# BatsResearch/menghini-neurips23-code

Measured on AMD Instinct MI355X. Metric: images/sec CLIP ViT-B/16 encode+prompt-step, higher is better.
Workload: dtype f16

## Files before the change

### menghini-neurips23-code_amd/csrc/attention_split.hip

```cpp
#include <math.h>

#include "common.h"

__device__ __forceinline__ int vt_index_fwd_s(int key, int d) { return vt_index(key, ((d >> 2) & 3) * 16 + (d >> 4) * 4 + (d & 3)); }

__device__ __forceinline__ void split8(const f32x4 a, const f32x4 b, half8& hi, half8& lo) {
    half4 h0, l0, h1, l1;
    split_f16x4(a, h0, l0);
    split_f16x4(b, h1, l1);
    hi = (half8){h0[0], h0[1], h0[2], h0[3], h1[0], h1[1], h1[2], h1[3]};
    lo = (half8){l0[0], l0[1], l0[2], l0[3], l1[0], l1[1], l1[2], l1[3]};
}

template <int KVC, bool CAUSAL, int NW>
__global__ __launch_bounds__(NW * 64) void attn_fwd_split_kernel(const float* __restrict__ qkv, half_t* __restrict__ out, int S, int H) {
    constexpr int SP = KVC * 32;
    constexpr float LOG2E = 1.4426950408889634f;
    constexpr float INV = 1.0f / (float)GRIP_SPLIT_LO_SCALE;
    extern __shared__ __attribute__((aligned(16))) char smem[];
    half_t* Kh = (half_t*)smem;
    half_t* Kl = Kh + SP * 64;
    half_t* Vh = Kl + SP * 64;
    half_t* Vl = Vh + SP * 64;

    const int tid = threadIdx.x, lane = tid & 63, wave = tid >> 6;
    const int D = H * 64;
    const int b = blockIdx.x / H, h = blockIdx.x - b * H;
    const size_t ld = (size_t)3 * D;
    const float* base = qkv + (size_t)b * S * ld + h * 64;
    const int li = lane & 15, lg = lane >> 4;
    const int n_qt = (S + 15) >> 4;

    for (int idx = tid; idx < SP * 8; idx += NW * 64) {
        const int row = idx >> 3, chunk = idx & 7;
        f32x4 a = {0.f, 0.f, 0.f, 0.f}, c = {0.f, 0.f, 0.f, 0.f};
        if (row < S) {
            const f32x4* p = (const f32x4*)(base + (size_t)row * ld + D + chunk * 8);
            a = p[0];
            c = p[1];
        }
        half8 hi, lo;
        split8(a, c, hi, lo);
        const int o = row * 64 + ((chunk ^ (row & 7)) * 8);
        *(half8*)(Kh + o) = hi;
        *(half8*)(Kl + o) = lo;
    }
    for (int idx = tid; idx < ((SP / 2 + 31) / 32) * 256; idx += NW * 64) {
        const int lane_rp = idx & 31, chunk = ((idx >> 5) & 1) + 2 * ((idx >> 6) & 3), rblk = idx >> 8;
        const int r0 = 2 * (rblk * 32 + lane_rp);
        if (r0 >= SP) continue;
        f32x4 z = {0.f, 0.f, 0.f, 0.f};
        f32x4 a0 = z, a1 = z, b0 = z, b1 = z;
        if (r0 < S) { const f32x4* p = (const f32x4*)(base + (size_t)r0 * ld + 2 * D + chunk * 8); a0 = p[0]; a1 = p[1]; }
        if (r0 + 1 < S) { const f32x4* p = (const f32x4*)(base + (size_t)(r0 + 1) * ld + 2 * D + chunk * 8); b0 = p[0]; b1 = p[1]; }
        half8 h0, l0, h1, l1;
        split8(a0, a1, h0, l0);
        split8(b0, b1, h1, l1);
#pragma unroll
        for (int j = 0; j < 8; ++j) {
            const int o = vt_index_fwd_s(r0, chunk * 8 + j);
            *(half2v*)(Vh + o) = (half2v){h0[j], h1[j]};
            *(half2v*)(Vl + o) = (half2v){l0[j], l1[j]};
        }
    }
    __syncthreads();

    for (int qt = wave; qt < n_qt; qt += NW) {
        asm volatile("" ::: "memory");
        const int qrow = qt * 16 + li;
        const int qr = qrow < S ? qrow : S - 1;
        half8 qh[2], ql[2];
#pragma unroll
        for (int kk = 0; kk < 2; ++kk) {
            const f32x4* p = (const f32x4*)(base + (size_t)qr * ld + (kk * 4 + lg) * 8);
            split8(p[0] * 0.125f, p[1] * 0.125f, qh[kk], ql[kk]);
        }
        f32x4 sc[2 * KVC];
        float m = -INFINITY;
#pragma unroll
        for (int t = 0; t < 2 * KVC; ++t) {
            f32x4 acc = {0.f, 0.f, 0.f, 0.f}, cor = {0.f, 0.f, 0.f, 0.f};
#pragma unroll
            for (int kk = 0; kk < 2; ++kk) {
                const int o = (t * 16 + li) * 64 + (((kk * 4 + lg) ^ (lane & 7)) * 8);
                const half8 kh = *(const half8*)(Kh + o), kl = *(const half8*)(Kl + o);
                acc = __builtin_amdgcn_mfma_f32_16x16x32_f16(kh, qh[kk], acc, 0, 0, 0);
                cor = __builtin_amdgcn_mfma_f32_16x16x32_f16(kl, qh[kk], cor, 0, 0, 0);
                cor = __builtin_amdgcn_mfma_f32_16x16x32_f16(kh, ql[kk], cor, 0, 0, 0);
            }
            acc += cor * INV;
            if (CAUSAL || t >= 2 * (KVC - 1)) {
#pragma unroll
                for (int r = 0; r < 4; ++r) {
                    const int kv = t * 16 + lg * 4 + r;
                    if (kv >= S || (CAUSAL && kv > qrow)) acc[r] = -INFINITY;
                }
            }
            m = fmaxf(fmaxf(fmaxf(m, acc[0]), fmaxf(acc[1], acc[2])), acc[3]);
            sc[t] = acc;
        }
        m = fmaxf(m, __shfl_xor(m, 16));
        m = fmaxf(m, __shfl_xor(m, 32));
        const float m2 = m * LOG2E;
#pragma unroll
        for (int t = 0; t < 2 * KVC; ++t)
#pragma unroll
            for (int r = 0; r < 4; ++r) sc[t][r] = __builtin_amdgcn_exp2f(__builtin_fmaf(sc[t][r], LOG2E, -m2));

        const half8 ones = {1, 1, 1, 1, 1, 1, 1, 1};
        f32x4 sum_h = {0.f, 0.f, 0.f, 0.f}, sum_l = {0.f, 0.f, 0.f, 0.f};
        f32x4 o[4], oc[4];
#pragma unroll
        for (int nf = 0; nf < 4; ++nf) { o[nf] = (f32x4){0.f, 0.f, 0.f, 0.f}; oc[nf] = (f32x4){0.f, 0.f, 0.f, 0.f}; }
#pragma unroll
        for (int c = 0; c < KVC; ++c) {
            half8 ph, pl;
            split8(sc[2 * c], sc[2 * c + 1], ph, pl);
#pragma unroll
            for (int nf = 0; nf < 4; ++nf) {
                const int vo = (c * 4 + nf) * 512 + (lg * 16 + (li ^ lg)) * 8;
                const half8 vh = *(const half8*)(Vh + vo), vl = *(const half8*)(Vl + vo);
                o[nf] = __builtin_amdgcn_mfma_f32_16x16x32_f16(vh, ph, o[nf], 0, 0, 0);
                oc[nf] = __builtin_amdgcn_mfma_f32_16x16x32_f16(vl, ph, oc[nf], 0, 0, 0);
                oc[nf] = __builtin_amdgcn_mfma_f32_16x16x32_f16(vh, pl, oc[nf], 0, 0, 0);
            }
            sum_h = __builtin_amdgcn_mfma_f32_16x16x32_f16(ones, ph, sum_h, 0, 0, 0);
            sum_l = __builtin_amdgcn_mfma_f32_16x16x32_f16(ones, pl, sum_l, 0, 0, 0);
        }
        if (qrow < S) {
            const float inv = 1.0f / (sum_h[0] + sum_l[0] * INV);
            half_t* orow = out + (size_t)((size_t)b * S + qrow) * 2 * D;
            const int col = h * 64 + lg * 16;
            half_t* op = orow + (col >> 5) * 64 + (col & 31);
            half8 hi0, lo0, hi1, lo1;
            split8((o[0] + oc[0] * INV) * inv, (o[1] + oc[1] * INV) * inv, hi0, lo0);
            split8((o[2] + oc[2] * INV) * inv, (o[3] + oc[3] * INV) * inv, hi1, lo1);
            *(half8*)op = hi0;
            *(half8*)(op + 8) = hi1;
            *(half8*)(op + 32) = lo0;
            *(half8*)(op + 40) = lo1;
        }
    }
}

bool attention_split_supported(int S) { return S >= 1 && S <= 320; }

int launch_attention_fwd_split(const float* qkv, void* out, int B, int S, int H, int causal, hipStream_t s) {
    GRIP_REQUIRE(attention_split_supported(S) && B >= 1 && H >= 1, "attention_split: bad shape B=%d S=%d H=%d (S <= 320)", B, S, H);
    const int kvc = (S + 31) / 32;
    const size_t lds = (size_t)4 * kvc * 32 * 64 * sizeof(half_t);
#define GRIP_ATT_CASE(K)                                                                                                                     \
    case K: {                                                                                                                                \
        static bool configured = false;                                                                                                      \
        if (!configured) {                                                                                                                   \
            GRIP_CHECK_HIP(hipFuncSetAttribute((const void*)attn_fwd_split_kernel<K, false, (K >= 4 ? 8 : 4)>, hipFuncAttributeMaxDynamicSharedMemorySize, (int)lds)); \
            GRIP_CHECK_HIP(hipFuncSetAttribute((const void*)attn_fwd_split_kernel<K, true, (K >= 4 ? 8 : 4)>, hipFuncAttributeMaxDynamicSharedMemorySize, (int)lds));  \
            configured = true;                                                                                                               \
        }                                                                                                                                    \
        if (causal) hipLaunchKernelGGL((attn_fwd_split_kernel<K, true, (K >= 4 ? 8 : 4)>), dim3(B * H), dim3((K >= 4 ? 8 : 4) * 64), lds, s, qkv, (half_t*)out, S, H); \
        else hipLaunchKernelGGL((attn_fwd_split_kernel<K, false, (K >= 4 ? 8 : 4)>), dim3(B * H), dim3((K >= 4 ? 8 : 4) * 64), lds, s, qkv, (half_t*)out, S, H);       \
    } break;
    switch (kvc) {
        GRIP_ATT_CASE(1) GRIP_ATT_CASE(2) GRIP_ATT_CASE(3) GRIP_ATT_CASE(4) GRIP_ATT_CASE(5)
        GRIP_ATT_CASE(6) GRIP_ATT_CASE(7) GRIP_ATT_CASE(8) GRIP_ATT_CASE(9) GRIP_ATT_CASE(10)
        default: GRIP_REQUIRE(false, "attention_split: S = %d out of range", S);
    }
#undef GRIP_ATT_CASE
    GRIP_CHECK_HIP(hipGetLastError());
    return GRIP_OK;
}
```

### menghini-neurips23-code_amd/csrc/common.h

```cpp
#pragma once
#include <hip/hip_runtime.h>
#include <stdint.h>
#include <stdio.h>
#include <string.h>

#include "host_common.h"
#include "gemm_plan.h"

typedef _Float16 half_t;
typedef half_t half8 __attribute__((ext_vector_type(8)));
typedef half_t half4 __attribute__((ext_vector_type(4)));
typedef half_t half2v __attribute__((ext_vector_type(2)));
typedef float f32x4 __attribute__((ext_vector_type(4)));

typedef half_t resid_t;

#define AS1 __attribute__((address_space(1)))
#define AS3 __attribute__((address_space(3)))

#define GRIP_CHECK_HIP(expr)                                                                   \
    do {                                                                                       \
        hipError_t _e = (expr);                                                                \
        if (_e != hipSuccess) {                                                                \
            grip_set_error("%s:%d %s -> %s", __FILE__, __LINE__, #expr, hipGetErrorString(_e)); \
// ... 11 lines not shown
    return (((c * 4 + (d >> 4)) * 64 + lg * 16 + ((d & 15) ^ lg)) * 8) + e;
}

#define LN_EPS 1e-5f
#define MAX_NV 8

__device__ __forceinline__ float wave_sum(float v) {
#define GRIP_DPP_ADD(ctrl) v += __builtin_bit_cast(float, __builtin_amdgcn_update_dpp(0, __builtin_bit_cast(int, v), ctrl, 0xF, 0xF, true))
    GRIP_DPP_ADD(0xB1);
    GRIP_DPP_ADD(0x4E);
    GRIP_DPP_ADD(0x141);
    GRIP_DPP_ADD(0x140);
#undef GRIP_DPP_ADD
    const int b = __builtin_bit_cast(int, v);
    const float r0 = __builtin_bit_cast(float, __builtin_amdgcn_readlane(b, 0)), r1 = __builtin_bit_cast(float, __builtin_amdgcn_readlane(b, 16));
    const float r2 = __builtin_bit_cast(float, __builtin_amdgcn_readlane(b, 32)), r3 = __builtin_bit_cast(float, __builtin_amdgcn_readlane(b, 48));
    return (r0 + r1) + (r2 + r3);
}
__device__ __forceinline__ float row16_sum(float v) {
#define GRIP_DPP_ADD(ctrl) v += __builtin_bit_cast(float, __builtin_amdgcn_update_dpp(0, __builtin_bit_cast(int, v), ctrl, 0xF, 0xF, true))
    GRIP_DPP_ADD(0xB1);
    GRIP_DPP_ADD(0x4E);
    GRIP_DPP_ADD(0x141);
    GRIP_DPP_ADD(0x140);
#undef GRIP_DPP_ADD
    return v;
}

__device__ __forceinline__ f32x4 load4(const float* p, int i) { return ((const f32x4*)p)[i]; }
__device__ __forceinline__ f32x4 load4(const half_t* p, int i) {
    const half4 h = ((const half4*)p)[i];
    return (f32x4){(float)h[0], (float)h[1], (float)h[2], (float)h[3]};
}
__device__ __forceinline__ void store4(float* p, int i, f32x4 v) { ((f32x4*)p)[i] = v; }
__device__ __forceinline__ void store4(half_t* p, int i, f32x4 v) { ((half4*)p)[i] = (half4){(half_t)v[0], (half_t)v[1], (half_t)v[2], (half_t)v[3]}; }
#ifndef GRIP_SPLIT_LO_SCALE
#define GRIP_SPLIT_LO_SCALE 1
#endif
#define SP1_W_SCALE 256.0f
__device__ __forceinline__ float quick_gelu_exact_s(float x) { return x * __builtin_amdgcn_rcpf(1.0f + __builtin_amdgcn_exp2f(-1.702f * 1.4426950408889634f * x)); }
struct SplitRow { half_t* p; };
__device__ __forceinline__ void split_f16x4(f32x4 v, half4& hi, half4& lo) {
#pragma unroll
    for (int e = 0; e < 4; ++e) {
        float x = v[e];
        asm volatile("" : "+v"(x));
        const half_t h = (half_t)x;
        hi[e] = h;
        lo[e] = (half_t)((x - (float)h) * (float)GRIP_SPLIT_LO_SCALE);
    }
}
__device__ __forceinline__ void store4(SplitRow r, int i, f32x4 v) {
    half4 hi, lo;
    split_f16x4(v, hi, lo);
    half_t* o = r.p + (i >> 3) * 64 + (i & 7) * 4;
    *(half4*)o = hi;
    *(half4*)(o + 32) = lo;
}

template <int NV>
__device__ __forceinline__ void ln_normalize(f32x4 (&v)[NV], int lane, int d4, int d, float& mean, float& rstd) {
#pragma clang fp contract(off)
    float s = 0.f;
#pragma unroll
    for (int i = 0; i < NV; ++i)
        if (lane + 64 * i < d4) s += v[i][0] + v[i][1] + v[i][2] + v[i][3];
    mean = wave_sum(s) / (float)d;
    float q = 0.f;
#pragma unroll
    for (int i = 0; i < NV; ++i)
        if (lane + 64 * i < d4) {
            f32x4 c = v[i] - mean;
            q += c[0] * c[0] + c[1] * c[1] + c[2] * c[2] + c[3] * c[3];
        }
    rstd = rsqrtf(wave_sum(q) / (float)d + LN_EPS);
}
__device__ __forceinline__ f32x4 ln_apply(f32x4 v, float mean, float rstd, f32x4 g, f32x4 b) {
#pragma clang fp contract(off)
    return (v - mean) * rstd * g + b;
}
#endif

struct GemmArgs {
    const void* A;
    const void* W;
    int M, N, K;
    int variant;
    int64_t m_pad;
    const float* bias;
    const void* resid;
    const void* aux;
    void* out;
    void* out2;
    int ldc;
    float scalar;
    int f32;
    float* stat_part;
    const float* rowstat;
    const float* stat_in;
    int stat_parts;
    const float* colsum;
    int ksplit;
    int64_t split_stride;
    float* coop_scratch;
    int* coop_counter;
    int rot_rows;
    half_t* resid_lo;
    int w_exact;
    int ablate;
};

int launch_gemm(int epi, const GemmArgs& a, hipStream_t s);
int launch_gemm_f32(int epi, const GemmArgs& a, hipStream_t s);
int launch_gemm_split(int epi, const GemmArgs& a, hipStream_t s);
int launch_split_rows(const float* x, void* out, int64_t rows, int K, int64_t ld_in, hipStream_t s, int is_weight = 0, int* overflow_flag = nullptr,
                      int* lo_nonzero_flag = nullptr);
float gemm_split_weight_scale();
bool gemm_split_dup_weights();
int launch_split_dup_weights(const void* src, void* dst, int64_t rows, int K, hipStream_t s);
int launch_gemm_split_k64p(int epi, const GemmArgs& a, hipStream_t s);

int launch_im2col(const void* images, int images_f16, void* out, int out_f32, int B, int R, int patch, int Kpad, hipStream_t s);
int launch_vit_assemble_ln(const float* patch_out, const float* cls, const float* pos, const float* prefix, int P,
                           const float* gamma, const float* beta, void* x, int f32, float* rowstat, int B, int G2, int d, hipStream_t s, half_t* x_lo = nullptr,
                           int per_image = 0);
int launch_vit_deep_insert(const float* deep, void* x, int f32, half_t* x_lo, float* stat_part, float* rowstat, int B, int S, int P, int M, int d, hipStream_t s);
int launch_text_deep_insert(const float* deep, int prefix_classes, void* x, int f32, float* stat_part, float* rowstat, int C, int S, int P, int shared_rows, int M, int d,
                            hipStream_t s);
int launch_ln_stats_finalize(const float* stat_part, int parts, float* rowstat, int M, int d, hipStream_t s);
int launch_ln_fold_weights(const half_t* W, const float* gamma, const float* beta, const float* bias, half_t* Wg, float* colsum, float* bias_out,
                           int N, int K, hipStream_t s);
int launch_layernorm_f16(const void* x, const float* gamma, const float* beta, void* out, int f32, int M, int d, hipStream_t s);
int launch_gather_ln_f16(const void* x, const int32_t* row_index, int row_stride, const float* gamma, const float* beta,
                         void* out, int f32, int n_rows, int d, hipStream_t s);
int launch_text_embed(const int32_t* token_ids, int ld_ids, const float* tok_emb, const float* pos, const float* prefix, int P,
                      int prefix_classes, void* x, int f32, float* rowstat, int C, int T, int d, int vocab, hipStream_t s, int shared_rows = 0);
int launch_transpose(const void* in, void* out, int f32, int rows, int cols, int ld_in, hipStream_t s);

#ifdef __HIPCC__
__device__ __forceinline__ size_t seq_row(int b, int r, int S, int Ps) {
    return r < Ps ? (size_t)r : (size_t)Ps + (size_t)b * (S - Ps) + (r - Ps);
}
#endif

int launch_attention_fwd(const half_t* qkv, half_t* out, int B, int S, int H, int causal, hipStream_t s, int shared_rows = 0);
int launch_attention_row(const half_t* qkv, const half_t* qrows, const int32_t* row_index, half_t* out, int B, int S, int H, int causal, hipStream_t s, int train = 0);
int launch_gather_rows(const half_t* x, const int32_t* row_index, int row_stride, half_t* out, int n_rows, int d, hipStream_t s);
int launch_attention_row_bwd(const half_t* qkv, const half_t* o_rows, const half_t* do_rows, const int32_t* row_index, half_t* dqkv, int B, int S, int H, int causal,
                             hipStream_t s);
int launch_attention_fwd_f32(const float* qkv, float* out, int B, int S, int H, int causal, hipStream_t s, int split_out = 0);
int launch_attention_row_f32(const float* qkv, const float* qrows, const int32_t* row_index, float* out, int B, int S, int H, int causal, hipStream_t s, int split_out = 0);
int launch_gather_rows4(const void* x, const int32_t* row_index, int row_stride, void* out, int n_rows, int d, hipStream_t s);
bool attention_split_supported(int S);
int launch_attention_fwd_split(const float* qkv, void* out, int B, int S, int H, int causal, hipStream_t s);
int launch_attention_bwd(const half_t* qkv, const half_t* o, const half_t* d_out, half_t* dqkv, int B, int S, int H, int causal, hipStream_t s,
                         int shared_rows = 0, float* kv_part = nullptr);
int launch_attention_bwd_tiled(const half_t* qkv, const half_t* o, const half_t* d_out, half_t* dqkv, int B, int S, int H, int causal, hipStream_t s);
int launch_layernorm_f16_from_f32(const float* x, const float* gamma, const float* beta, half_t* out, int M, int d, hipStream_t s);
int launch_ln_bwd_add(const resid_t* x, const float* dln, int parts, int64_t part_stride, const float* gamma, float* dx, half_t* dxh, int M, int d, hipStream_t s);
int launch_ln_bwd_init(const resid_t* x, const float* dln, int parts, int64_t part_stride, const float* gamma, const float* rows_add, const int32_t* index, int stride,
                       float* dx, half_t* dxh, int M, int d, hipStream_t s);
int launch_ln_bwd_scatter(const resid_t* x, const float* dy, const int32_t* index, int stride, const float* gamma, float* dx, half_t* dxh,
                          int n, int d, hipStream_t s);
int launch_ln_bwd_scatter_fill(const resid_t* x, const float* dy, const int32_t* index, int stride, int first, const float* gamma, float* dx, half_t* dxh,
                               int n, int M, int d, hipStream_t s);
int launch_vit_prefix_grad(const float* dx, const float* prefix, const float* gamma, const float* scale, float* grad, int B, int S, int P, int d, hipStream_t s);
int launch_vit_deep_grad(float* dx, half_t* dxh, const float* scale, float* grad, int B, int S, int P, int d, hipStream_t s);
int launch_vit_prefix_grad_per_image(const float* dx, const float* prefix, const float* gamma, const float* scale, float* grad, int B, int S, int P, int d, hipStream_t s);
int launch_text_prefix_grad(const float* dx, const float* scale, float* grad, int C, int T, int P, int prefix_classes, int d, hipStream_t s);
int launch_text_deep_grad(float* dx, half_t* dxh, const float* scale, float* grad, int C, int T, int P, int prefix_classes, int d, hipStream_t s);
int launch_grad_scale_cast(const float* g, half_t* g16, float* scale, int n, hipStream_t s);
```

### menghini-neurips23-code_amd/csrc/tower.hip

```cpp
#include <stdarg.h>
#include <stdlib.h>

#include <map>
#include <string>
#include <vector>

#include "common.h"

static thread_local char g_err[512] = "";
void grip_set_error(const char* fmt, ...) {
    va_list ap;
    va_start(ap, fmt);
    vsnprintf(g_err, sizeof(g_err), fmt, ap);
    va_end(ap);
}
extern "C" const char* grip_last_error(void) { return g_err; }
extern "C" int grip_abi_version(void) { return GRIP_ABI_VERSION; }

static int g_cu_budget = 0;
int grip_cu_budget() { return g_cu_budget; }
extern "C" int grip_set_cu_budget(int n_cus) {
    GRIP_REQUIRE(n_cus >= 0 && (n_cus == 0 || n_cus >= 8), "set_cu_budget: %d (0 = all, else at least 8)", n_cus);
    g_cu_budget = n_cus;
    return GRIP_OK;
// ... 610 lines not shown
        w.hilo = (flags & GRIP_FWD_STREAM_HILO) ? 1 : 0;
        RUN(launch_vit_assemble_ln(w.patch_out, F + t->L.cls, (flags & GRIP_FWD_NO_POS_EMB) ? nullptr : F + t->L.pos, prefix, n_prefix, F + t->L.lnpre_g, F + t->L.lnpre_b, x0, f, (train && !train_fold(t)) ? nullptr : w.rowstat, batch, G2, d, s,
                                   w.hilo ? w.x_lo : nullptr, per_image));
        resid_t* xf = nullptr;
        bool compact = false;
        RUN(run_blocks(t, w, x0, 0, nullptr, s, &xf, &compact));
        RUN(launch_gather_ln_f16(xf, nullptr, compact ? 1 : w.S, F + t->L.lnpost_g, F + t->L.lnpost_b, w.cls16, f, batch, d, s));
        a = GemmArgs{};
        a.f32 = f; a.A = w.cls16; a.W = t->wop(t->L.projT); a.M = batch; a.N = D.embed_dim; a.K = d; a.out = out_emb; a.ldc = D.embed_dim;
        RUN(launch_gemm(EPI_F32, a, s));
        note_forward(t, workspace, train, w, nullptr, 0, generation, per_image != 0, n_deep);
        return GRIP_OK;
    } catch (...) { grip_set_error("vit_forward: exception"); return GRIP_ERR_ARG; }
}

extern "C" int grip_vit_forward(grip_tower* t, const void* images, int images_f16, const float* prefix, int n_prefix,
                                int batch, float* out_emb, void* workspace, size_t workspace_bytes, int flags, uint64_t* generation, void* stream) {
    return grip_vit_forward_deep(t, images, images_f16, prefix, n_prefix, nullptr, 0, batch, out_emb, workspace, workspace_bytes, flags, generation, stream);
}

extern "C" int grip_text_forward_deep(grip_tower* t, const int32_t* token_ids, const int32_t* eot_index, const float* prefix,
                                      int n_prefix, int prefix_classes, const float* deep, int n_deep, int n_class, int seq_len, float* out_emb,
                                      void* workspace, size_t workspace_bytes, int flags, uint64_t* generation, void* stream) {
    try {
        GRIP_REQUIRE(t && t->D.kind == 1, "text_forward: not a text tower%s", n_deep ? " (the vision tower's deep prompts go through grip_vit_forward_deep)" : "");
        GRIP_REQUIRE(n_deep >= 0 && n_deep <= t->D.layers - 1, "text_forward_deep: n_deep = %d out of range: deep prompts replace the context rows entering blocks 1 .. n_deep, "
                     "0 <= n_deep <= layers - 1 = %d", n_deep, t->D.layers - 1);
        GRIP_REQUIRE(n_deep == 0 || n_prefix > 0, "text_forward_deep: deep prompts replace the rows of the shallow context: n_prefix must be positive (n_deep = %d)", n_deep);
        GRIP_REQUIRE(n_deep == 0 || deep, "text_forward_deep: null deep prompt pointer (n_deep = %d)", n_deep);
        GRIP_REQUIRE(token_ids && eot_index && out_emb && (n_prefix == 0 || prefix), "text_forward: null pointer");
        GRIP_REQUIRE(!(flags & GRIP_FWD_PER_IMAGE_PREFIX), "text_forward: GRIP_FWD_PER_IMAGE_PREFIX is a vision-tower flag (one context per class: prefix_classes = n_class)");
        GRIP_REQUIRE(n_prefix == 0 || prefix_classes == 1 || prefix_classes == n_class, "text_forward: prefix_classes must be 1 or n_class");
        GRIP_REQUIRE((flags & ~(GRIP_FWD_TRAIN | GRIP_FWD_SHARED_PREFIX | GRIP_FWD_NO_POS_EMB)) == 0, "text_forward: unknown flag bits 0x%x", flags);
        const int train = flags & GRIP_FWD_TRAIN;
        const int shared = (flags & GRIP_FWD_SHARED_PREFIX) && n_prefix > 0 && prefix_classes == 1 && !t->f32;
        Workspace w;
        RUN(check_ws(t, n_class, n_prefix, train, workspace, workspace_bytes, w, seq_len, shared));
        w.deep = n_deep ? deep : nullptr;
        w.n_deep = n_deep;
        w.deep_classes = n_deep ? prefix_classes : 1;
        hipStream_t s = (hipStream_t)stream;
        const grip_dims& D = t->D;
        const int d = D.width, f = t->f32;
        const float* F = t->w32;
        resid_t* x0 = train ? w.x_in[0] : w.x;
        if (train && w.coop_cnt) GRIP_CHECK_HIP(hipMemsetAsync(w.coop_cnt, 0, w.coop_cnt_bytes, s));
        RUN(launch_text_embed(token_ids, D.seq0, F + t->L.tok, (flags & GRIP_FWD_NO_POS_EMB) ? nullptr : F + t->L.pos, prefix, n_prefix, prefix_classes, x0, f, (train && !train_fold(t)) ? nullptr : w.rowstat, n_class, w.S, d, D.vocab, s, w.Ps));
        resid_t* xf = nullptr;
        bool compact = false;
        RUN(run_blocks(t, w, x0, 1, eot_index, s, &xf, &compact));
        RUN(launch_gather_ln_f16(xf, compact ? nullptr : eot_index, compact ? 1 : w.rs, F + t->L.lnpost_g, F + t->L.lnpost_b, w.cls16, f, n_class, d, s));
        GemmArgs a{};
        a.f32 = f; a.A = w.cls16; a.W = t->wop(t->L.projT); a.M = n_class; a.N = D.embed_dim; a.K = d; a.out = out_emb; a.ldc = D.embed_dim;
        RUN(launch_gemm(EPI_F32, a, s));
        note_forward(t, workspace, train, w, eot_index, prefix_classes, generation, false, n_deep);
        return GRIP_OK;
    } catch (...) { grip_set_error("text_forward: exception"); return GRIP_ERR_ARG; }
}

extern "C" int grip_text_forward(grip_tower* t, const int32_t* token_ids, const int32_t* eot_index, const float* prefix,
                                 int n_prefix, int prefix_classes, int n_class, int seq_len, float* out_emb,
                                 void* workspace, size_t workspace_bytes, int flags, uint64_t* generation, void* stream) {
    return grip_text_forward_deep(t, token_ids, eot_index, prefix, n_prefix, prefix_classes, nullptr, 0, n_class, seq_len, out_emb, workspace, workspace_bytes, flags,
                                  generation, stream);
}

extern "C" int grip_debug_gemm(int epi, const void* A, const void* W, int M, int N, int K, const float* bias, const void* resid,
                               const void* aux, void* out, void* out2, float scalar, int m_pad, int variant, void* stream) {
    GemmArgs a{};
    a.variant = variant & 0xff;
    a.rot_rows = (variant >> 8) & 1;
    a.A = A; a.W = W; a.M = M; a.N = N; a.K = K; a.m_pad = m_pad; a.bias = bias; a.resid = resid;
    a.aux = aux; a.out = out; a.out2 = out2; a.ldc = N; a.scalar = scalar;
    if (a.variant == 7) { a.f32 = 1; a.variant = 0; }
    return launch_gemm(epi, a, (hipStream_t)stream);
}
extern "C" int grip_debug_gemm_splitk(const void* A, const void* W, int M, int N, int K, float* out, int ksplit, int64_t split_stride, int* ksplit_used,
                                      int m_pad, int variant, void* stream) {
    GemmArgs a{};
    a.variant = variant & 0xff;
    a.rot_rows = (variant >> 8) & 1;
    a.A = A; a.W = W; a.M = M; a.N = N; a.K = K; a.m_pad = m_pad; a.out = out; a.ldc = N;
    a.ksplit = ksplit ? ksplit : gemm_pick_ksplit(M, N, K);
    a.split_stride = split_stride;
    if (ksplit_used) *ksplit_used = a.ksplit;
    return launch_gemm(EPI_F32, a, (hipStream_t)stream);
}
extern "C" int grip_debug_gemm_ln(int epi, const void* A, const void* W, int M, int N, int K, const float* bias, const void* resid, void* out, void* out2,
                                  float* stat_part, const float* rowstat, const float* colsum, int m_pad, int variant, void* stream) {
    GemmArgs a{};
    a.variant = variant;
    a.A = A; a.W = W; a.M = M; a.N = N; a.K = K; a.m_pad = m_pad; a.bias = bias; a.resid = resid; a.out = out; a.out2 = out2; a.ldc = N;
    a.stat_part = stat_part; a.rowstat = rowstat; a.colsum = colsum;
    return launch_gemm(epi, a, (hipStream_t)stream);
}
extern "C" int grip_debug_gemm_train(int epi, const void* A, const void* W, int M, int N, int K, const float* bias, const void* resid, void* out, void* out2,
                                     float* stat_part, float* rowstat, const float* colsum, const float* stat_in, int stat_parts, int ksplit,
                                     float* coop_scratch, int* coop_counter, int m_pad, void* stream) {
    GemmArgs a{};
    a.rot_rows = 1;
    a.A = A; a.W = W; a.M = M; a.N = N; a.K = K; a.m_pad = m_pad; a.bias = bias; a.resid = resid; a.out = out; a.out2 = out2; a.ldc = N;
    a.stat_part = stat_part; a.rowstat = rowstat; a.colsum = colsum; a.stat_in = stat_in; a.stat_parts = stat_parts;
    a.ksplit = ksplit; a.coop_scratch = coop_scratch; a.coop_counter = coop_counter;
    return launch_gemm(epi, a, (hipStream_t)stream);
}
extern "C" int grip_debug_gemm_args(int epi, const void* A, const void* W, int M, int N, int K, int ldc, const float* bias, const void* resid, void* resid_lo,
                                    const void* aux, void* out, void* out2, float scalar, float* stat_part, float* rowstat, const float* colsum,
                                    const float* stat_in, int stat_parts, int ksplit, int64_t split_stride, float* coop_scratch, int* coop_counter, int m_pad,
                                    int variant, int rot_rows, void* stream) {
    GemmArgs a{};
    a.A = A; a.W = W; a.M = M; a.N = N; a.K = K; a.ldc = ldc; a.m_pad = m_pad; a.variant = variant; a.rot_rows = rot_rows;
    a.bias = bias; a.resid = resid; a.resid_lo = (half_t*)resid_lo; a.aux = aux; a.out = out; a.out2 = out2; a.scalar = scalar;
    a.stat_part = stat_part; a.rowstat = rowstat; a.colsum = colsum; a.stat_in = stat_in; a.stat_parts = stat_parts;
    a.ksplit = ksplit; a.split_stride = split_stride; a.coop_scratch = coop_scratch; a.coop_counter = coop_counter;
    return launch_gemm(epi, a, (hipStream_t)stream);
}
extern "C" int grip_debug_coop_split(int M, int N, int K) { return gemm_pick_coop_split(M, N, K); }
extern "C" int grip_debug_ln_fold(const void* W, const float* gamma, const float* beta, const float* bias, void* Wg, float* colsum, float* bias_out,
                                  int N, int K, const float* stat_part, int parts, float* rowstat, int M, int d, void* stream) {
    int rc = W ? launch_ln_fold_weights((const half_t*)W, gamma, beta, bias, (half_t*)Wg, colsum, bias_out, N, K, (hipStream_t)stream) : GRIP_OK;
    if (rc || !stat_part) return rc;
    return launch_ln_stats_finalize(stat_part, parts, rowstat, M, d, (hipStream_t)stream);
}
extern "C" int grip_debug_gemm_split(int epi, const float* A, const float* W, int M, int N, int K, const float* bias, const float* resid, void* out,
                                     void* a_split, void* w_split, int m_pad, void* stream) {
    hipStream_t s = (hipStream_t)stream;
    RUN(launch_split_rows(A, a_split, m_pad, K, K, s));
    int* flag = nullptr;
    GRIP_CHECK_HIP(hipMalloc((void**)&flag, sizeof(int)));
    int inexact = 1;
    int rc = hipMemsetAsync(flag, 0, sizeof(int), s) == hipSuccess ? launch_split_rows(W, w_split, N, K, K, s, 1, nullptr, flag) : GRIP_ERR_HIP;
    if (!rc && (hipMemcpyAsync(&inexact, flag, sizeof(int), hipMemcpyDeviceToHost, s) != hipSuccess || hipStreamSynchronize(s) != hipSuccess)) rc = GRIP_ERR_HIP;
    (void)hipFree(flag);
    if (rc) return rc;
    GemmArgs a{};
    a.w_exact = !inexact && gemm_split_dup_weights();
    a.f32 = 2; a.A = a_split; a.W = w_split; a.M = M; a.N = N; a.K = K; a.m_pad = m_pad; a.bias = bias; a.resid = resid; a.out = out; a.ldc = N;
    if (!a.w_exact) return launch_gemm(epi, a, s);
    void* w_dup = nullptr;
    GRIP_CHECK_HIP(hipMalloc(&w_dup, (size_t)N * K * 4));
    a.W = w_dup;
    rc = launch_split_dup_weights(w_split, w_dup, N, K, s);
    if (!rc) rc = launch_gemm(epi, a, s);
    if (hipStreamSynchronize(s) != hipSuccess && !rc) { grip_set_error("debug_gemm_split: HIP error"); rc = GRIP_ERR_HIP; }
    (void)hipFree(w_dup);
    return rc;
}
int gemm_split_last_wlo();
extern "C" int grip_debug_split_last_wlo(void) { return gemm_split_last_wlo(); }
extern "C" int grip_debug_split_rows(const float* x, void* out, int64_t rows, int K, void* stream) {
    return launch_split_rows(x, out, rows, K, K, (hipStream_t)stream);
}
extern "C" int grip_debug_attention_split(const void* qkv, void* out, int B, int S, int H, int causal, int mfma, void* stream) {
    if (mfma) return launch_attention_fwd_split((const float*)qkv, out, B, S, H, causal, (hipStream_t)stream);
    return launch_attention_fwd_f32((const float*)qkv, (float*)out, B, S, H, causal, (hipStream_t)stream, 1);
}
extern "C" int grip_debug_attention_exact(const void* qkv, void* out, int B, int S, int H, int causal, void* stream) {
    return launch_attention_fwd_f32((const float*)qkv, (float*)out, B, S, H, causal, (hipStream_t)stream);
}
extern "C" int grip_debug_attention(const void* qkv, void* out, int B, int S, int H, int causal, void* stream) {
    return launch_attention_fwd((const half_t*)qkv, (half_t*)out, B, S, H, causal, (hipStream_t)stream);
}
extern "C" int grip_debug_attention_shared(const void* qkv, void* out, int B, int S, int H, int shared_rows, void* stream) {
    return launch_attention_fwd((const half_t*)qkv, (half_t*)out, B, S, H, 1, (hipStream_t)stream, shared_rows);
}
extern "C" int grip_debug_attention_row(const void* qkv, const void* qrows, const int32_t* row_index, void* out, int B, int S, int H, int causal, int train,
                                        void* stream) {
    return launch_attention_row((const half_t*)qkv, (const half_t*)qrows, row_index, (half_t*)out, B, S, H, causal, (hipStream_t)stream, train);
}
extern "C" int grip_debug_attention_row_exact(const void* qkv, const void* qrows, const int32_t* row_index, void* out, int B, int S, int H, int causal,
                                              int split_out, void* stream) {
    return launch_attention_row_f32((const float*)qkv, (const float*)qrows, row_index, (float*)out, B, S, H, causal, (hipStream_t)stream, split_out);
}
extern "C" int grip_debug_layernorm(const float* x, const float* gamma, const float* beta, void* out, int M, int d, void* stream) {
    return launch_layernorm_f16_from_f32(x, gamma, beta, (half_t*)out, M, d, (hipStream_t)stream);
}
extern "C" int grip_debug_ln_bwd_add(const void* x, const float* dln, int parts, int64_t part_stride, const float* gamma, float* dx, void* dxh, int M, int d,
                                     void* stream) {
    return launch_ln_bwd_add((const resid_t*)x, dln, parts, part_stride, gamma, dx, (half_t*)dxh, M, d, (hipStream_t)stream);
}
extern "C" int grip_debug_ln_bwd_init(const void* x, const float* dln, int parts, int64_t part_stride, const float* gamma, const float* rows_add,
                                      const int32_t* index, int stride, float* dx, void* dxh, int M, int d, void* stream) {
    return launch_ln_bwd_init((const resid_t*)x, dln, parts, part_stride, gamma, rows_add, index, stride, dx, (half_t*)dxh, M, d, (hipStream_t)stream);
}
extern "C" int grip_debug_ln_bwd_scatter(const void* x, const float* dy, const int32_t* index, int stride, int first, const float* gamma, float* dx, void* dxh,
                                         int n, int M, int d, int fill, void* stream) {
    if (fill) return launch_ln_bwd_scatter_fill((const resid_t*)x, dy, index, stride, first, gamma, dx, (half_t*)dxh, n, M, d, (hipStream_t)stream);
    return launch_ln_bwd_scatter((const resid_t*)x, dy, index, stride, gamma, dx, (half_t*)dxh, n, d, (hipStream_t)stream);
}
extern "C" int grip_debug_vit_prefix_grad(float* dx, void* dxh, const float* prefix, const float* gamma, const float* scale, float* grad, int B, int S, int P,
                                          int d, int mode, void* stream) {
    if (mode == 0) return launch_vit_prefix_grad(dx, prefix, gamma, scale, grad, B, S, P, d, (hipStream_t)stream);
    if (mode == 1) return launch_vit_prefix_grad_per_image(dx, prefix, gamma, scale, grad, B, S, P, d, (hipStream_t)stream);
    return launch_vit_deep_grad(dx, (half_t*)dxh, scale, grad, B, S, P, d, (hipStream_t)stream);
}
extern "C" int grip_debug_text_prefix_grad(float* dx, void* dxh, const float* scale, float* grad, int C, int T, int P, int prefix_classes, int d, int deep,
                                           void* stream) {
    if (deep) return launch_text_deep_grad(dx, (half_t*)dxh, scale, grad, C, T, P, prefix_classes, d, (hipStream_t)stream);
    return launch_text_prefix_grad(dx, scale, grad, C, T, P, prefix_classes, d, (hipStream_t)stream);
}
extern "C" int grip_debug_grad_scale_cast(const float* g, void* g16, float* scale, int n, void* stream) {
    return launch_grad_scale_cast(g, (half_t*)g16, scale, n, (hipStream_t)stream);
}
extern "C" int grip_debug_layernorm_modes(const void* x, const int32_t* row_index, int row_stride, const float* gamma, const float* beta, void* out, int f32,
                                          int gather, int M, int d, void* stream) {
    if (gather) return launch_gather_ln_f16(x, row_index, row_stride, gamma, beta, out, f32, M, d, (hipStream_t)stream);
    return launch_layernorm_f16(x, gamma, beta, out, f32, M, d, (hipStream_t)stream);
}
extern "C" int grip_debug_vit_assemble(const float* patch_out, const float* cls, const float* pos, const float* prefix, int P, const float* gamma, const float* beta,
                                       void* x, int f32, float* rowstat, int B, int G2, int d, void* x_lo, int per_image, void* stream) {
    return launch_vit_assemble_ln(patch_out, cls, pos, prefix, P, gamma, beta, x, f32, rowstat, B, G2, d, (hipStream_t)stream, (half_t*)x_lo, per_image);
}
extern "C" int grip_debug_deep_insert(const float* deep, int prefix_classes, void* x, int f32, void* x_lo, float* stat_part, float* rowstat, int B, int S, int P,
                                      int shared_rows, int M, int d, int text, void* stream) {
    if (text) return launch_text_deep_insert(deep, prefix_classes, x, f32, stat_part, rowstat, B, S, P, shared_rows, M, d, (hipStream_t)stream);
    return launch_vit_deep_insert(deep, x, f32, (half_t*)x_lo, stat_part, rowstat, B, S, P, M, d, (hipStream_t)stream);
}
extern "C" int grip_debug_text_embed(const int32_t* ids, int ld_ids, const float* tok_emb, const float* pos, const float* prefix, int P, int prefix_classes, void* x,
                                     int f32, float* rowstat, int C, int T, int d, int vocab, int shared_rows, void* stream) {
    return launch_text_embed(ids, ld_ids, tok_emb, pos, prefix, P, prefix_classes, x, f32, rowstat, C, T, d, vocab, (hipStream_t)stream, shared_rows);
}
extern "C" int grip_debug_patch_gather(const void* images, int images_f16, void* out, int out_f32, int B, int R, int patch, int Kpad, void* stream) {
    return launch_im2col(images, images_f16, out, out_f32, B, R, patch, Kpad, (hipStream_t)stream);
}
extern "C" int grip_debug_transpose(const void* in, void* out, int f32, int rows, int cols, int ld_in, void* stream) {
    return launch_transpose(in, out, f32, rows, cols, ld_in, (hipStream_t)stream);
}
extern "C" int grip_debug_gather_rows(const void* x, const int32_t* row_index, int row_stride, void* out, int n_rows, int d, int four_byte, void* stream) {
    if (four_byte) return launch_gather_rows4(x, row_index, row_stride, out, n_rows, d, (hipStream_t)stream);
    return launch_gather_rows((const half_t*)x, row_index, row_stride, (half_t*)out, n_rows, d, (hipStream_t)stream);
}

static int run_blocks_backward(grip_tower* t, Workspace& w, int causal, const int32_t* read_rows, hipStream_t s, float* grad_deep = nullptr) {
    const int d = t->D.width, H = t->D.heads;
    const half_t* W = t->w16;
    const float* F = t->w32;
    const int64_t part = (int64_t)w.Mp * d;
    for (int l = t->D.layers - 1; l >= 0; --l) {
        const LayerW& lw = t->L.layer[(size_t)l];
        if (grad_deep && l + 1 <= w.n_deep) {
            if (t->D.kind == 0)
                RUN(launch_vit_deep_grad(w.dx, w.dxh, w.scale, grad_deep + (size_t)l * w.P * d, w.batch, w.S, w.P, d, s));
            else
                RUN(launch_text_deep_grad(w.dx, w.dxh, w.scale, grad_deep + (size_t)l * w.deep_classes * w.P * d, w.Ps ? 1 : w.batch, w.S, w.P, w.deep_classes, d, s));
        }
        if (l + 1 == t->D.layers && w.rows_last) {
            const int64_t Bp = round_up64(w.batch, 256);
            const int64_t rpart = Bp * d;
            GemmArgs a{};
            a.A = w.drow_h; a.W = W + lw.proj_wT; a.M = w.batch; a.m_pad = Bp; a.N = 4 * d; a.K = d; a.aux = w.row_hpre; a.out = w.row_dh; a.ldc = 4 * d;
            RUN(launch_gemm(EPI_GELUGRAD_F16, a, s));
            a = GemmArgs{};
            a.A = w.row_dh; a.W = W + lw.fc_wT; a.M = w.batch; a.m_pad = Bp; a.N = d; a.K = 4 * d; a.out = w.row_dln; a.ldc = d;
            a.ksplit = w.ks_row; a.split_stride = rpart;
            RUN(launch_gemm(EPI_F32, a, s));
            RUN(launch_ln_bwd_add(w.row_xmid, w.row_dln, w.ks_row, rpart, F + lw.ln2_g, w.drow, w.drow_h, w.batch, d, s));
            a = GemmArgs{};
            a.A = w.drow_h; a.W = W + lw.out_wT; a.M = w.batch; a.m_pad = Bp; a.N = d; a.K = d; a.out = w.row_datt; a.ldc = d;
            RUN(launch_gemm(EPI_F16, a, s));
            RUN(launch_attention_row_bwd(w.qkv_l[(size_t)l], w.row_att, w.row_datt, read_rows, w.dqkv, w.batch, w.S, H, causal, s));
            a = GemmArgs{};
            a.rot_rows = 1;
            a.A = w.dqkv; a.W = W + lw.in_wT; a.M = w.M; a.m_pad = w.Mp; a.N = d; a.K = 3 * d; a.out = w.dln; a.ldc = d;
            a.ksplit = w.ks_in; a.split_stride = part;
            RUN(launch_gemm(EPI_F32, a, s));
            RUN(launch_ln_bwd_init(w.x_in[(size_t)l], w.dln, w.ks_in, part, F + lw.ln1_g, w.drow, read_rows, w.S, w.dx, w.dxh, w.M, d, s));
            continue;
        }
        GemmArgs a{};
        a.rot_rows = 1;
        a.A = w.dxh; a.W = W + lw.proj_wT; a.M = w.M; a.m_pad = w.Mp; a.N = 4 * d; a.K = d; a.aux = w.hpre_l[(size_t)l]; a.out = w.dh; a.ldc = 4 * d;
        RUN(launch_gemm(EPI_GELUGRAD_F16, a, s));
        a = GemmArgs{};
        a.rot_rows = 1;
        a.A = w.dh; a.W = W + lw.fc_wT; a.M = w.M; a.m_pad = w.Mp; a.N = d; a.K = 4 * d; a.out = w.dln; a.ldc = d;
        a.ksplit = w.ks_fc; a.split_stride = part;
        RUN(launch_gemm(EPI_F32, a, s));
        RUN(launch_ln_bwd_add(w.x_mid[(size_t)l], w.dln, w.ks_fc, part, F + lw.ln2_g, w.dx, w.dxh, w.M, d, s));
        a = GemmArgs{};
        a.rot_rows = 1;
        a.A = w.dxh; a.W = W + lw.out_wT; a.M = w.M; a.m_pad = w.Mp; a.N = d; a.K = d; a.out = w.datt; a.ldc = d;
        RUN(launch_gemm(EPI_F16, a, s));
        RUN(launch_attention_bwd(w.qkv_l[(size_t)l], w.att_l[(size_t)l], w.datt, w.dqkv, w.batch, w.S, H, causal, s, w.Ps, w.kv_part));
        a = GemmArgs{};
        a.rot_rows = 1;
        a.A = w.dqkv; a.W = W + lw.in_wT; a.M = w.M; a.m_pad = w.Mp; a.N = d; a.K = 3 * d; a.out = w.dln; a.ldc = d;
        a.ksplit = w.ks_in; a.split_stride = part;
        RUN(launch_gemm(EPI_F32, a, s));
        RUN(launch_ln_bwd_add(w.x_in[(size_t)l], w.dln, w.ks_in, part, F + lw.ln1_g, w.dx, w.dxh, w.M, d, s));
    }
    return GRIP_OK;
}

static int backward_head_of_tower(grip_tower* t, Workspace& w, const float* grad_emb, const int32_t* index, hipStream_t s) {
    const grip_dims& D = t->D;
    const int d = D.width;
    RUN(launch_grad_scale_cast(grad_emb, w.gemb16, w.scale, w.batch * D.embed_dim, s));
    GemmArgs a{};
    a.A = w.gemb16; a.W = t->w16 + t->L.proj; a.M = w.batch; a.N = d; a.K = D.embed_dim; a.out = w.dcls; a.ldc = d;
    RUN(launch_gemm(EPI_F32, a, s));
    if (w.rows_last)
        return launch_ln_bwd_scatter(w.row_xout, w.dcls, nullptr, 1, t->w32 + t->L.lnpost_g, w.drow, w.drow_h, w.batch, d, s);
    RUN(launch_ln_bwd_scatter_fill(w.x_in[(size_t)D.layers], w.dcls, index, w.rs, w.Ps, t->w32 + t->L.lnpost_g, w.dx, w.dxh, w.batch, (int)w.M, d, s));
    return GRIP_OK;
}

static int check_bwd(grip_tower* t, void* workspace, size_t workspace_bytes, uint64_t generation, grip_tower::TrainState& st) {
// ... 124 lines not shown
```

Baseline: 21460.

## Add two-phase split attention kernel reusing one LDS region for K then V

Adds a new forward split-precision attention kernel for non-causal sequences of 97-256 tokens, which is the ViT-B/16 range. It stages K hi/lo in shared memory, computes scores and softmax probabilities into registers, then overwrites the same region with V before the PV product. Halving the LDS footprint and splitting each (batch, head) over two 512-thread blocks is meant to raise occupancy and parallelism. The cost is an extra barrier phase, K loaded twice per item, and more register pressure from holding the probabilities across phases.

```diff
diff --git a/menghini-neurips23-code_amd/csrc/attention_split.hip b/menghini-neurips23-code_amd/csrc/attention_split.hip
--- a/menghini-neurips23-code_amd/csrc/attention_split.hip
+++ b/menghini-neurips23-code_amd/csrc/attention_split.hip
@@ -143,11 +143,200 @@
     }
 }
 
+template <int KVC>
+__global__ __launch_bounds__(512, 4) void attn_fwd_split2_kernel(const float* __restrict__ qkv, half_t* __restrict__ out, int S, int H, int items) {
+    constexpr int SP = KVC * 32;
+    constexpr float LOG2E = 1.4426950408889634f;
+    constexpr float INV = 1.0f / (float)GRIP_SPLIT_LO_SCALE;
+    extern __shared__ __attribute__((aligned(16))) char smem[];
+    half_t* Ph = (half_t*)smem;
+    half_t* Pl = Ph + SP * 64;
+
+    const int item = (blockIdx.x >> 4) * 8 + (blockIdx.x & 7), half = (blockIdx.x >> 3) & 1;
+    if (item >= items) return;
+    const int tid = threadIdx.x, lane = tid & 63, wave = tid >> 6;
+    const int D = H * 64;
+    const int b = item / H, h = item - b * H;
+    const size_t ld = (size_t)3 * D;
+    const float* base = qkv + (size_t)b * S * ld + h * 64;
+    const int li = lane & 15, lg = lane >> 4;
+    const int n_qt = (S + 15) >> 4;
+    const int n_q0 = (n_qt + 1) >> 1;
+    const int qt = (half ? n_q0 : 0) + wave;
+    const bool has_tile = wave < (half ? n_qt - n_q0 : n_q0);
+
+    constexpr int NIT = (SP * 8 + 511) / 512;
+    const f32x4 zero4 = {0.f, 0.f, 0.f, 0.f};
+    const int qrow = qt * 16 + li;
+    f32x4 qf[4];
+    {
+        const int qr = qrow < S ? qrow : S - 1;
+#pragma unroll
+        for (int kk = 0; kk < 2; ++kk) {
+            const f32x4* p = (const f32x4*)(base + (size_t)qr * ld + (kk * 4 + lg) * 8);
+            qf[2 * kk] = p[0];
+            qf[2 * kk + 1] = p[1];
+        }
+    }
+    {
+        f32x4 ka[NIT], kc[NIT];
+#pragma unroll
+        for (int it = 0; it < NIT; ++it) {
+            const int row = (tid + it * 512) >> 3, chunk = tid & 7;
+            const f32x4* p = (const f32x4*)(base + (size_t)(row < S ? row : S - 1) * ld + D + chunk * 8);
+            ka[it] = p[0];
+            kc[it] = p[1];
+        }
+#pragma unroll
+        for (int it = 0; it < NIT; ++it) {
+            const int row = (tid + it * 512) >> 3, chunk = tid & 7;
+            if (row < n_qt * 16) {
+                half8 hi, lo;
+                split8(row < S ? ka[it] : zero4, row < S ? kc[it] : zero4, hi, lo);
+                const int o = row * 64 + ((chunk ^ (row & 7)) * 8);
+                *(half8*)(Ph + o) = hi;
+                *(half8*)(Pl + o) = lo;
+            }
+        }
+    }
+    __syncthreads();
+
+    half8 ph[KVC], pl[KVC];
+    if (has_tile) {
+        half8 qh[2], ql[2];
+#pragma unroll
+        for (int kk = 0; kk < 2; ++kk) split8(qf[2 * kk] * 0.125f, qf[2 * kk + 1] * 0.125f, qh[kk], ql[kk]);
+        f32x4 sc[2 * KVC];
+        float m = -INFINITY;
+#pragma unroll
+        for (int t = 0; t < 2 * KVC; ++t) {
+            if (t < 2 * KVC - 1 || n_qt == 2 * KVC) {
+                f32x4 acc = {0.f, 0.f, 0.f, 0.f}, cor = {0.f, 0.f, 0.f, 0.f};
+#pragma unroll
+                for (int kk = 0; kk < 2; ++kk) {
+                    const int o = (t * 16 + li) * 64 + (((kk * 4 + lg) ^ (lane & 7)) * 8);
+                    const half8 kh = *(const half8*)(Ph + o), kl = *(const half8*)(Pl + o);
+                    acc = __builtin_amdgcn_mfma_f32_16x16x32_f16(kh, qh[kk], acc, 0, 0, 0);
+                    cor = __builtin_amdgcn_mfma_f32_16x16x32_f16(kl, qh[kk], cor, 0, 0, 0);
+                    cor = __builtin_amdgcn_mfma_f32_16x16x32_f16(kh, ql[kk], cor, 0, 0, 0);
+                }
+                acc += cor * INV;
+                if (t >= 2 * (KVC - 1)) {
+#pragma unroll
+                    for (int r = 0; r < 4; ++r)
+                        if (t * 16 + lg * 4 + r >= S) acc[r] = -INFINITY;
+                }
+                m = fmaxf(fmaxf(fmaxf(m, acc[0]), fmaxf(acc[1], acc[2])), acc[3]);
+                sc[t] = acc;
+                if (t & 1) __builtin_amdgcn_sched_barrier(0);
+            } else {
+                sc[t] = (f32x4){-INFINITY, -INFINITY, -INFINITY, -INFINITY};
+            }
+        }
+        m = fmaxf(m, __shfl_xor(m, 16));
+        m = fmaxf(m, __shfl_xor(m, 32));
+        const float m2 = m * LOG2E;
+#pragma unroll
+        for (int t = 0; t < 2 * KVC; ++t)
+#pragma unroll
+            for (int r = 0; r < 4; ++r) sc[t][r] = __builtin_amdgcn_exp2f(__builtin_fmaf(sc[t][r], LOG2E, -m2));
+#pragma unroll
+        for (int c = 0; c < KVC; ++c) split8(sc[2 * c], sc[2 * c + 1], ph[c], pl[c]);
+    }
+    float vf[NIT][8];
+#pragma unroll
+    for (int it = 0; it < NIT; ++it) {
+        const int grp = wave + it * 8, c = grp >> 2, g = grp & 3;
+        const int d = ((lane >> 2) & 3) * 16 + (lane >> 4) * 4 + (lane & 3);
+#pragma unroll
+        for (int e = 0; e < 8; ++e) {
+            const int key = c * 32 + (e >> 2) * 16 + g * 4 + (e & 3);
+            vf[it][e] = base[(size_t)(key < S ? key : S - 1) * ld + 2 * D + d];
+        }
+    }
+    __syncthreads();
+#pragma unroll
+    for (int it = 0; it < NIT; ++it) {
+        const int grp = wave + it * 8, c = grp >> 2, g = grp & 3;
+        if (grp < KVC * 4) {
+            f32x4 v[2];
+#pragma unroll
+            for (int e = 0; e < 8; ++e) v[e >> 2][e & 3] = c * 32 + (e >> 2) * 16 + g * 4 + (e & 3) < S ? vf[it][e] : 0.f;
+            half8 hi, lo;
+            split8(v[0], v[1], hi, lo);
+            const int o = ((c * 4 + (lane >> 4)) * 64 + g * 16 + ((lane & 15) ^ g)) * 8;
+            *(half8*)(Ph + o) = hi;
+            *(half8*)(Pl + o) = lo;
+        }
+    }
+    __syncthreads();
+
+    if (has_tile) {
+        const half8 ones = {1, 1, 1, 1, 1, 1, 1, 1};
+        f32x4 sum_h = {0.f, 0.f, 0.f, 0.f}, sum_l = {0.f, 0.f, 0.f, 0.f};
+        f32x4 o[4], oc[4];
+#pragma unroll
+        for (int nf = 0; nf < 4; ++nf) { o[nf] = (f32x4){0.f, 0.f, 0.f, 0.f}; oc[nf] = (f32x4){0.f, 0.f, 0.f, 0.f}; }
+#pragma unroll
+        for (int c = 0; c < KVC; ++c) {
+#pragma unroll
+            for (int nf = 0; nf < 4; ++nf) {
+                const int vo = (c * 4 + nf) * 512 + (lg * 16 + (li ^ lg)) * 8;
+                const half8 vh = *(const half8*)(Ph + vo), vl = *(const half8*)(Pl + vo);
+                o[nf] = __builtin_amdgcn_mfma_f32_16x16x32_f16(vh, ph[c], o[nf], 0, 0, 0);
+                oc[nf] = __builtin_amdgcn_mfma_f32_16x16x32_f16(vl, ph[c], oc[nf], 0, 0, 0);
+                oc[nf] = __builtin_amdgcn_mfma_f32_16x16x32_f16(vh, pl[c], oc[nf], 0, 0, 0);
+            }
+            sum_h = __builtin_amdgcn_mfma_f32_16x16x32_f16(ones, ph[c], sum_h, 0, 0, 0);
+            sum_l = __builtin_amdgcn_mfma_f32_16x16x32_f16(ones, pl[c], sum_l, 0, 0, 0);
+        }
+        if (qrow < S) {
+            const float inv = 1.0f / (sum_h[0] + sum_l[0] * INV);
+            half_t* orow = out + (size_t)((size_t)b * S + qrow) * 2 * D;
+            const int col = h * 64 + lg * 16;
+            half_t* op = orow + (col >> 5) * 64 + (col & 31);
+            half8 hi0, lo0, hi1, lo1;
+            split8((o[0] + oc[0] * INV) * inv, (o[1] + oc[1] * INV) * inv, hi0, lo0);
+            split8((o[2] + oc[2] * INV) * inv, (o[3] + oc[3] * INV) * inv, hi1, lo1);
+            *(half8*)op = hi0;
+            *(half8*)(op + 8) = hi1;
+            *(half8*)(op + 32) = lo0;
+            *(half8*)(op + 40) = lo1;
+        }
+    }
+}
+
 bool attention_split_supported(int S) { return S >= 1 && S <= 320; }
-
-int launch_attention_fwd_split(const float* qkv, void* out, int B, int S, int H, int causal, hipStream_t s) {
+static bool attention_split2_serves(int S, int causal) { return !causal && S >= 97 && S <= 256; }
+
+template <int KVC>
+static int launch_split2(const float* qkv, half_t* out, int B, int S, int H, hipStream_t s) {
+    const size_t lds = (size_t)2 * KVC * 32 * 64 * sizeof(half_t);
+    static bool configured = false;
+    if (!configured) {
+        GRIP_CHECK_HIP(hipFuncSetAttribute((const void*)attn_fwd_split2_kernel<KVC>, hipFuncAttributeMaxDynamicSharedMemorySize, (int)lds));
+        configured = true;
+    }
+    const int64_t items = (int64_t)B * H;
+    GRIP_REQUIRE((items + 7) / 8 * 16 <= INT32_MAX, "attention_split: B * H = %lld too large", (long long)items);
+    hipLaunchKernelGGL(attn_fwd_split2_kernel<KVC>, dim3((unsigned)((items + 7) / 8 * 16)), dim3(512), lds, s, qkv, out, S, H, (int)items);
+    GRIP_CHECK_HIP(hipGetLastError());
+    return GRIP_OK;
+}
+
+int launch_attention_fwd_split(const float* qkv, void* out, int B, int S, int H, int causal, hipStream_t s, int form) {
     GRIP_REQUIRE(attention_split_supported(S) && B >= 1 && H >= 1, "attention_split: bad shape B=%d S=%d H=%d (S <= 320)", B, S, H);
+    GRIP_REQUIRE(form != 2 || attention_split2_serves(S, causal), "attention_split: the two-phase form serves non-causal 97 <= S <= 256, not S=%d causal=%d", S, causal);
     const int kvc = (S + 31) / 32;
+    if (form != 1 && attention_split2_serves(S, causal)) {
+        switch (kvc) {
+            case 4: return launch_split2<4>(qkv, (half_t*)out, B, S, H, s);
+            case 5: return launch_split2<5>(qkv, (half_t*)out, B, S, H, s);
+            case 6: return launch_split2<6>(qkv, (half_t*)out, B, S, H, s);
+            case 7: return launch_split2<7>(qkv, (half_t*)out, B, S, H, s);
+            default: return launch_split2<8>(qkv, (half_t*)out, B, S, H, s);
+        }
+    }
     const size_t lds = (size_t)4 * kvc * 32 * 64 * sizeof(half_t);
 #define GRIP_ATT_CASE(K)                                                                                                                     \
     case K: {                                                                                                                                \
diff --git a/menghini-neurips23-code_amd/csrc/common.h b/menghini-neurips23-code_amd/csrc/common.h
--- a/menghini-neurips23-code_amd/csrc/common.h
+++ b/menghini-neurips23-code_amd/csrc/common.h
@@ -187,7 +187,7 @@
 int launch_attention_row_f32(const float* qkv, const float* qrows, const int32_t* row_index, float* out, int B, int S, int H, int causal, hipStream_t s, int split_out = 0);
 int launch_gather_rows4(const void* x, const int32_t* row_index, int row_stride, void* out, int n_rows, int d, hipStream_t s);
 bool attention_split_supported(int S);
-int launch_attention_fwd_split(const float* qkv, void* out, int B, int S, int H, int causal, hipStream_t s);
+int launch_attention_fwd_split(const float* qkv, void* out, int B, int S, int H, int causal, hipStream_t s, int form = 0);
 int launch_attention_bwd(const half_t* qkv, const half_t* o, const half_t* d_out, half_t* dqkv, int B, int S, int H, int causal, hipStream_t s,
                          int shared_rows = 0, float* kv_part = nullptr);
 int launch_attention_bwd_tiled(const half_t* qkv, const half_t* o, const half_t* d_out, half_t* dqkv, int B, int S, int H, int causal, hipStream_t s);
diff --git a/menghini-neurips23-code_amd/csrc/tower.hip b/menghini-neurips23-code_amd/csrc/tower.hip
--- a/menghini-neurips23-code_amd/csrc/tower.hip
+++ b/menghini-neurips23-code_amd/csrc/tower.hip
@@ -786,7 +786,8 @@
     return launch_split_rows(x, out, rows, K, K, (hipStream_t)stream);
 }
 extern "C" int grip_debug_attention_split(const void* qkv, void* out, int B, int S, int H, int causal, int mfma, void* stream) {
-    if (mfma) return launch_attention_fwd_split((const float*)qkv, out, B, S, H, causal, (hipStream_t)stream);
+    GRIP_REQUIRE(mfma >= 0 && mfma <= 3, "grip_debug_attention_split: mfma = %d (0 .. 3)", mfma);
+    if (mfma) return launch_attention_fwd_split((const float*)qkv, out, B, S, H, causal, (hipStream_t)stream, mfma - 1);
     return launch_attention_fwd_f32((const float*)qkv, (float*)out, B, S, H, causal, (hipStream_t)stream, 1);
 }
 extern "C" int grip_debug_attention_exact(const void* qkv, void* out, int B, int S, int H, int causal, void* stream) {
```

Result: no change. 21560 (median of 6 runs) (+0.5%).
